# Nablax/Path-Tracer-CUDA-OpenGL

Hardware: AMD Instinct MI355X
Metric: Mray/s + ms/frame, bunny-in-Cornell 1920×1080 @1024spp, 1/2/4/8 MI355X (higher is better)
Workload: dtype f32

## Files before the change

### path-tracer-cuda-opengl_amd/csrc/pt_device.hip

```cpp
#include <hip/hip_runtime.h>

#include <algorithm>
#include <array>
#include <atomic>
#include <chrono>
#include <cfloat>
#include <cmath>
#include <cstdio>
#include <cstdlib>
#include <cstring>
#include <limits>
#include <type_traits>
#include <memory>
#include <string>
#include <vector>

#include "../host/pt_error.hpp"
#include "../host/pt_host.hpp"
#include "../host/pt_inst_dev.hpp"
#include "../host/pt_wide8.hpp"
#include "../host/pt_wide_dev.hpp"
#include "pt.h"
#include "pt_math.hpp"

// ... 55 lines not shown
    uint32_t rays, visits, tris, spheres;
};

__device__ __forceinline__ float3 f3(float a, float b, float c) { return make_float3(a, b, c); }
__device__ __forceinline__ float3 add(float3 a, float3 b) { return f3(a.x + b.x, a.y + b.y, a.z + b.z); }
__device__ __forceinline__ float3 sub(float3 a, float3 b) { return f3(a.x - b.x, a.y - b.y, a.z - b.z); }
__device__ __forceinline__ float3 mul(float3 a, float3 b) { return f3(a.x * b.x, a.y * b.y, a.z * b.z); }
__device__ __forceinline__ float3 scale(float t, float3 v) { return f3(t * v.x, t * v.y, t * v.z); }
__device__ __forceinline__ float3 neg(float3 v) { return f3(-v.x, -v.y, -v.z); }
__device__ __forceinline__ float dot3(float3 a, float3 b) { return a.x * b.x + a.y * b.y + a.z * b.z; }
__device__ __forceinline__ float3 cross3(float3 u, float3 v) {
    return f3(u.y * v.z - u.z * v.y, u.z * v.x - u.x * v.z, u.x * v.y - u.y * v.x);
}
__device__ __forceinline__ float len2(float3 v) { return v.x * v.x + v.y * v.y + v.z * v.z; }
__device__ __forceinline__ float3 divs(float3 v, float t) { return scale(rcpRN(t), v); }
__device__ __forceinline__ float3 normalize3(float3 v) {
    float l = sqrtf(len2(v));
    if (l == 0.0f) return f3(0.0f, 0.0f, 0.0f);
    return divs(v, l);
}
__device__ __forceinline__ float3 xyz(float4 v) { return f3(v.x, v.y, v.z); }

struct Xorwow {
    uint32_t d, v0, v1, v2, v3, v4;
    __device__ __forceinline__ uint32_t next() {
        uint32_t t = v0 ^ (v0 >> 2);
        v0 = v1; v1 = v2; v2 = v3; v3 = v4;
        v4 = __builtin_amdgcn_bitop3_b32(v4, v4 << 4, t ^ (t << 1), 0x96);
        d += 362437u;
        return v4 + d;
    }
    __device__ __forceinline__ float uniform() { return uniformOf(next()); }
    __device__ __forceinline__ float centered2() { return centered2Of(uniform()); }
};

__device__ __forceinline__ Xorwow sampleStream(uint32_t k0, uint32_t k1, uint32_t sample, uint32_t pixel) {
    uint32_t c0 = sample, c1 = pixel, c2 = 0u, c3 = 0x53414D50u;
#pragma unroll 2
    for (int r = 0; r < 10; r++) {
        const uint64_t p0 = (uint64_t)0xD2511F53u * c0, p1 = (uint64_t)0xCD9E8D57u * c2;
        const uint32_t hi0 = (uint32_t)(p0 >> 32), lo0 = (uint32_t)p0;
        const uint32_t hi1 = (uint32_t)(p1 >> 32), lo1 = (uint32_t)p1;
        const uint32_t n0 = __builtin_amdgcn_bitop3_b32(hi1, c1, k0, 0x96), n2 = __builtin_amdgcn_bitop3_b32(hi0, c3, k1, 0x96);
        c0 = n0; c1 = lo1; c2 = n2; c3 = lo0;
        k0 += 0x9E3779B9u;
        k1 += 0xBB67AE85u;
    }
    return Xorwow{c3, c0, c1, c2, c3 ^ 0x6C078965u, c0 ^ c1 ^ 0x2545F491u};
}

struct SlabHit { bool hit; float lo; };

__host__ __device__ constexpr int nodeBoxIdx(int child, int axis, int isMax) { return 6 * child + 2 * axis + isMax; }

typedef float v2f __attribute__((ext_vector_type(2)));

__device__ __forceinline__ SlabHit slabPair(v2f X, v2f Y, v2f Z, float3 o, float3 inv, float tmin, float tmax) {
    const v2f tx = (X - o.x) * inv.x, ty = (Y - o.y) * inv.y, tz = (Z - o.z) * inv.z;
    float nx = inv.x < 0.0f ? tx.y : tx.x, fx = inv.x < 0.0f ? tx.x : tx.y;
    float ny = inv.y < 0.0f ? ty.y : ty.x, fy = inv.y < 0.0f ? ty.x : ty.y;
    float nz = inv.z < 0.0f ? tz.y : tz.x, fz = inv.z < 0.0f ? tz.x : tz.y;
    float lo = fmaxf(fmaxf(fmaxf(tmin, nx), ny), nz);
    float hi = fminf(fminf(fminf(tmax, fx), fy), fz);
    return SlabHit{!(hi < lo), lo};
}
struct SlabHit2 { SlabHit l, r; };
// ... 438 lines not shown
    const float4 s0 = r[0], s1 = r[1], s2 = r[2];
    const uint32_t tf = __float_as_uint(s2.y);
    const bool ident = __float_as_uint(ex.y) == 1u, linIdent = __float_as_uint(ex.y) != 0u;
    HitRec h;
    h.p = add(o, scale(t, d));
    float3 outward;
    if (tf >> 16) {
        const float3 po = ident ? h.p : xformPoint(r0, r1, r2, h.p);
        outward = divs(sub(po, xyz(s0)), s0.w);
    } else {
        outward = xyz(s0);
    }
    if (!linIdent) {
        const float3 n = outward;
        outward = normalize3(f3((r0.x * n.x + r1.x * n.y) + r2.x * n.z, (r0.y * n.x + r1.y * n.y) + r2.y * n.z,
                                (r0.z * n.x + r1.z * n.y) + r2.z * n.z));
    }
    h.front = dot3(d, outward) < 0.0f;
    h.n = h.front ? outward : neg(outward);
    h.mat = (int)__float_as_uint(s2.z);
    obj = (int)(__float_as_uint(ex.x) + __float_as_uint(s2.w));
    h.obj = obj;
    h.m0 = s1;
    h.ir = s2.x;
    h.type = (int)(tf & 0xffffu);
    return h;
}

template <class G>
__device__ __forceinline__ float3 onUnitSphere(G& g) {
    float3 res;
    float norm;
    do {
        const float a = g.centered2();
        const float b = g.centered2();
        const float cz = g.centered2();
        res = f3(a, b, cz);
        norm = len2(res);
    } while (norm >= 1.0f);
    return divs(res, sqrtf(norm));
}
template <class G>
__device__ __forceinline__ float3 inUnitSphere(G& g) {
    float3 res;
    do {
        const float a = g.centered2();
        const float b = g.centered2();
        const float cz = g.centered2();
        res = f3(a, b, cz);
    } while (len2(res) >= 1.0f);
    return res;
}
__device__ __forceinline__ float3 reflect3(float3 v, float3 n) { return sub(v, scale(2.0f * dot3(v, n), n)); }

template <class G>
__device__ __forceinline__ bool scatter(const DevScene& S, const HitRec& h, float3& d, float3& atten, G& g) {
    (void)S;
    const float4 m0 = h.m0;
    const int type = h.type;
    if (type == PT_LAMBERTIAN) {
        float3 dir = add(h.n, onUnitSphere(g));
        if (fabsf(dir.x) < 1e-7f && fabsf(dir.y) < 1e-7f && fabsf(dir.z) < 1e-7f) dir = h.n;
        d = dir;
        atten = xyz(m0);
        return true;
    }
    if (type == PT_METAL) {
        float3 refl = reflect3(normalize3(d), h.n);
        float3 fz = inUnitSphere(g);
        d = add(refl, scale(m0.w, fz));
        atten = xyz(m0);
        return dot3(d, h.n) > 0.0f;
    }
    if (type == PT_DIELECTRIC) {
        atten = f3(1.0f, 1.0f, 1.0f);
        const float ir = h.ir;
        float ratio = h.front ? rcpRN(ir) : ir;
        float3 ud = normalize3(d);
        float cos_t = fminf(dot3(neg(ud), h.n), 1.0f);
        float sin_t = sqrtf(1.0f - cos_t * cos_t);
        bool cannot = ratio * sin_t > 1.0f;
        bool refl = cannot;
// ... 308 lines not shown
#endif
#ifndef PT_LDS_STACK
#define PT_LDS_STACK 32
#endif
template <int STACK, bool SAMPLE, bool WIDE>
constexpr int kLdsStack = (!WIDE && STACK > PT_LDS_STACK) ? PT_LDS_STACK : STACK;
#ifndef PT_WIDE_SPEC
#define PT_WIDE_SPEC 1
#endif
#ifndef PT_WIDE_MIX
#define PT_WIDE_MIX 1
#endif
#ifndef PT_WIDE_WAVES_PER_EU
#define PT_WIDE_WAVES_PER_EU 5
#endif
#ifndef PT_COMPAT_WIDE_WAVES_PER_EU
#define PT_COMPAT_WIDE_WAVES_PER_EU 4
#endif
template <int STACK, bool SAMPLE, bool WIDE>
constexpr int kWavesPerEU = WIDE ? (SAMPLE || STACK > 8 ? PT_WIDE_WAVES_PER_EU : PT_COMPAT_WIDE_WAVES_PER_EU)
                                 : kLdsStack<STACK, SAMPLE, WIDE> <= 24
                                ? (SAMPLE ? PT_WAVES_PER_EU : 5)
                                : (kLdsStack<STACK, SAMPLE, WIDE> <= 32
                                       ? 5
                                       : (kLdsStack<STACK, SAMPLE, WIDE> <= 48 ? 4 : (STACK <= 64 ? 3 : 2)));

typedef const __attribute__((address_space(4))) RenderParams* KArgs;
__device__ __forceinline__ KArgs kargs() {
    KArgs k = (KArgs)__builtin_amdgcn_kernarg_segment_ptr();
    asm volatile("" : "+s"(k));
    return k;
}

typedef const __attribute__((address_space(4))) float KFloat;
typedef const __attribute__((address_space(4))) uint32_t* KU32;
__device__ __forceinline__ float3 ld3(const __attribute__((address_space(4))) float3& v) {
    KFloat* f = (KFloat*)&v;
    return f3(f[0], f[1], f[2]);
}
__device__ __forceinline__ DevScene ldScene(KArgs k) {
    DevScene S;
    S.nodes = k->S.nodes; S.prims = k->S.prims; S.shade = k->S.shade; S.mats = k->S.mats;
    S.wnodes = k->S.wnodes; S.wprims = k->S.wprims; S.wshade = k->S.wshade; S.wbox = k->S.wbox; S.rankOf = k->S.rankOf;
    S.iparent = k->S.iparent; S.err = k->S.err; S.nprims = k->S.nprims;
    S.hasSpheres = k->S.hasSpheres;
    S.cx = k->S.cx; S.cy = k->S.cy; S.cz = k->S.cz; S.ext = k->S.ext;
    S.mixLim = k->S.mixLim;
    S.winst = k->S.winst; S.gBits = k->S.gBits;
    return S;
}

template <bool LIT>
__device__ __forceinline__ float3 skyK(float3 d, float3 att) {
    if constexpr (LIT) return sky(d, att, ld3(kargs()->skyH), ld3(kargs()->skyZ));
    else return sky(d, att);
}

template <int STACK, bool SAMPLE, bool WIDE, bool INST = false, bool LIT = false>
__global__ __launch_bounds__(kWave) __attribute__((amdgpu_waves_per_eu(kWavesPerEU<STACK, SAMPLE, WIDE>))) void renderKernelWF(RenderParams P) {
    constexpr int LS = kLdsStack<STACK, SAMPLE, WIDE>;
    __shared__ uint32_t stk[LS * kWave];
    constexpr int SPECN = WIDE && !INST ? PT_WIDE_SPEC : 0;
    constexpr bool SPEC = SPECN > 0;
    __shared__ uint32_t pend[SPEC ? 2 * SPECN * kWave : 1];
    __shared__ float wray[INST ? 6 * kWave : 1];
    __shared__ uint4 taskState[SAMPLE ? kWave : 1];
// ... 38 lines not shown
    float fcol = (float)col;
    float frow = valid ? (float)globalRow(lrow, P.stripe_h, P.nparts, P.part) : 0.0f;
    const DevScene& S = P.S;
    const __amdgpu_buffer_rsrc_t nodeRsrc = rawRsrc(WIDE ? (const void*)S.wnodes : (const void*)S.nodes);
    uint32_t* my = stk + lane;
    uint32_t sRays = 0, sVisits = 0, sTris = 0, sSph = 0, sPaths = 0;
#ifdef PT_DIAG
    uint32_t itN = 0, itL = 0, itS = 0, sPops = 0, sRedo = 0;
    uint32_t sRedoMiss = 0;
    unsigned long long sSpecN = 0, sIdleN = 0;
    unsigned long long sHalf = 0, sParkT = 0;
    unsigned long long cycN = 0, cycL = 0, cycS = 0, cycH = 0;
    unsigned long long cycSh = 0, cycTk = 0, cycNp = 0, cycBr = 0;
#define PT_DIAG_ADD(v, x) (v) += (x)
#else
#define PT_DIAG_ADD(v, x) ((void)0)
#endif

    Xorwow g{};
    if constexpr (!SAMPLE) {
        if (valid) g = Xorwow{P.sd[idx], P.s0[idx], P.s1[idx], P.s2[idx], P.s3[idx], P.s4[idx]};
    }
    float3 sum = f3(0.0f, 0.0f, 0.0f), o = f3(0.0f, 0.0f, 0.0f), d = f3(0.0f, 0.0f, 1.0f);
    float3 inv = d, att = f3(1.0f, 1.0f, 1.0f);
    float closest = 0.0f;
    int best = -1, depthLeft = 0, sample = 0, node = -1, sp = 0, qn = 0;
    constexpr int LQ = (SAMPLE && !WIDE && STACK <= 32) ? PT_LEAF_QUEUE_SAMPLE : kLeafQ;
    uint32_t qref[LQ];
    float lq[LQ];
#pragma unroll
    for (int i = 0; i < LQ; i++) { qref[i] = 0u; lq[i] = 0.0f; }
    uint32_t ng = 0u, tgBase = 0u, tg = 0u, oct = 0u;
    float bestLo = 0.0f;
    bool active = false;
    uint32_t depthPaths = 0;
    uint32_t pxRays = 0;
    bool needTask = SAMPLE;
    uint32_t poolBase = 0u, poolLeft = 0u;


#define PT_BEGIN_RAY()                                                                              \
    do {                                                                                          \
        depthLeft--;                                                                              \
        if constexpr (SAMPLE) {    \
            if (kargs()->measureCost)                                                             \
                __hip_atomic_fetch_add(&taskState[lane].w, 1u, __ATOMIC_RELAXED, __HIP_MEMORY_SCOPE_WORKGROUP); \
        }                                                                                         \
        closest = __builtin_inff();                                                               \
        best = -1;                                                                                \
        sp = 0;                                                                                   \
        qn = 0;                                                                                   \
        if constexpr (CRITK) pxRays++;                                                            \
        if constexpr (WIDE) {                 \
            inv = f3(rcpRN(d.x), rcpRN(d.y), rcpRN(d.z));                                         \
            const uint32_t oc_ = (inv.x < 0.0f ? 1u : 0u) | (inv.y < 0.0f ? 2u : 0u) | (inv.z < 0.0f ? 4u : 0u); \
            oct = oc_;                                                                            \
            tg = 0u;                                                                              \
                    \
            bestLo = INST || kargs()->S.hasSpheres ? -__builtin_inff() : __builtin_inff();         \
            ng = S.nprims > 0 ? (1u << oc_) : 0u;                                                 \
                 \
            if (!INST && ((kargs()->camFar && depthLeft + 1 == kargs()->max_depth) ||              \
                          (PT_WIDE_MIX && mixUnsafe(inv, kargs()->S.mixLim)))) {                   \
                ng = 0u;             \
                oct |= 8u;      \
            }                                                                                     \
            if (INST && kargs()->camFar && depthLeft + 1 == kargs()->max_depth) {                  \
                     \
                const auto& K_ = *kargs();                                                        \
                (void)instEntry(K_.S.cx, K_.S.cy, K_.S.cz, K_.S.ext, o, d, inv);                   \
// ... 26 lines not shown
                sTris += (uint32_t)__popcll(__ballot(!isS_));                                     \
                sSph += (uint32_t)__popcll(__ballot(isS_));                                       \
                if (sph_) wideTest<true>(q_, o, d, inv, 0.001f, closest, best, bestLo, lb_, redo_, 0u); \
                else if (INST) wideTest<false>(q_, o, d, inv, 0.001f, closest, best, bestLo, lb_, redo_, 0u); \
                else wideTestTri(q_, o, d, 0.001f, closest, best, bestLo);    \
            }                                                                                     \
            if ((ng & 0xffu) == 0u) {                                                             \
                if (sp == 0) break;                                                               \
                sp--;                                                                             \
                ng = my[sp * kWave];                                                              \
            }                                                                                     \
            const uint32_t bit_ = (uint32_t)__builtin_ctz(ng & 0xffu);                            \
            const uint32_t child_ = (ng >> 8) + (bit_ ^ (oct & 7u));                              \
            ng &= ~(1u << bit_);                                                                  \
            if (ng & 0xffu) { my[sp * kWave] = ng; sp++; }    \
            sVisits += (uint32_t)__popcll(__ballot(true));                                        \
            const uint32_t off_ = mul80(child_);                                                  \
            const uint4 n0_ = __builtin_bit_cast(uint4, __builtin_amdgcn_raw_buffer_load_b128(nodeRsrc, off_, 0, 0)); \
            const uint4 n1_ = __builtin_bit_cast(uint4, __builtin_amdgcn_raw_buffer_load_b128(nodeRsrc, off_ + 16u, 0, 0)); \
            const uint4 n2_ = __builtin_bit_cast(uint4, __builtin_amdgcn_raw_buffer_load_b128(nodeRsrc, off_ + 32u, 0, 0)); \
            const uint4 n3_ = __builtin_bit_cast(uint4, __builtin_amdgcn_raw_buffer_load_b128(nodeRsrc, off_ + 48u, 0, 0)); \
            const uint4 n4_ = __builtin_bit_cast(uint4, __builtin_amdgcn_raw_buffer_load_b128(nodeRsrc, off_ + 64u, 0, 0)); \
            const uint32_t h_ = wideHits<PT_WIDE_MIX != 0>(n0_, n1_, n2_, n3_, n4_, o, inv, oct & 7u, 0.001f, closest); \
            ng = (n1_.x << 8) | (h_ >> 24);                                                      \
            tgBase = n1_.y;                                                                       \
            tg = h_ & 0xffffffu;                                                                  \
        }                                                                                         \
        if (redo_) oct |= 8u;              \
    } while (0)
#define PT_TAKE_TASKS(got)                                                                          \
    do {                                                                                          \
        const auto& Q_ = *kargs();                                                                \
        for (;;) {                                                                                \
            const uint64_t m_ = __ballot(needTask);                                               \
            if (m_ == 0) break;                                                                   \
            if (poolLeft == 0u) {  \
                const int leader_ = __ffsll((unsigned long long)m_) - 1;                          \
                          \
                const uint32_t grab_ = (uint32_t)kTaskPool;                                       \
                uint32_t b_ = 0;                                                                  \
                if (lane == leader_) b_ = atomicAdd(Q_.taskCounter, grab_);                       \
                poolBase = __builtin_amdgcn_readfirstlane((uint32_t)__shfl((int)b_, leader_));    \
                poolLeft = grab_;                                                                 \
            }                                                                                     \
              \
            const uint32_t base_ = poolBase;                                                      \
            const uint32_t take_ = min((uint32_t)__popcll(m_), poolLeft);                         \
            poolBase += take_;                                                                    \
            poolLeft -= take_;                                                                    \
            const uint32_t g0_ = base_ >> 6, off_ = base_ & 63u;                                  \
            const uint32_t slotA_ = Q_.nblocksShift >= 0 ? g0_ >> Q_.nblocksShift : g0_ / (uint32_t)Q_.ngroups; \
            const uint32_t blkA_ = g0_ - slotA_ * (uint32_t)Q_.ngroups;                           \
            const bool wrap_ = blkA_ + 1u == (uint32_t)Q_.ngroups;                                  \
            const uint32_t slotB_ = wrap_ ? slotA_ + 1u : slotA_, blkB_ = wrap_ ? 0u : blkA_ + 1u; \
            const uint32_t nslots_ = (uint32_t)Q_.ntiles;                                          \
             \
                                                    \
            const uint32_t xyA_ = slotA_ < nslots_ ? ((KU32)Q_.tileXY)[__builtin_amdgcn_readfirstlane(slotA_)] : 0u; \
            const uint32_t xyB_ = slotB_ < nslots_ ? ((KU32)Q_.tileXY)[__builtin_amdgcn_readfirstlane(slotB_)] : 0u; \
            const uint32_t txA_ = xyA_ & 0xffffu, tyA_ = xyA_ >> 16;                              \
            const uint32_t txB_ = xyB_ & 0xffffu, tyB_ = xyB_ >> 16;                              \
            const uint32_t k_ = (uint32_t)__popcll(m_ & ((1ull << lane) - 1ull));                 \
            if (needTask && k_ < take_) {                                                         \
                if (base_ + k_ >= Q_.ntasks) {                                                     \
                    needTask = false;                                                             \
                } else {                                                                          \
                    const uint32_t o_ = off_ + k_, px_ = o_ & 63u;                                \
                    const bool hi_ = o_ >= 64u;                                                   \
                    const int c_ = (int)((hi_ ? txB_ : txA_) * 8u + (px_ & 7u));                  \
                    const int r_ = (int)((hi_ ? tyB_ : tyA_) * 8u + (px_ >> 3));                  \
                    if (c_ < Q_.width && r_ < Q_.nrows) {                                           \
                        needTask = false;                                                         \
                        got = true;                                                               \
                        const uint32_t s0_ = (hi_ ? blkB_ : blkA_) * (uint32_t)Q_.span;           \
                        taskState[lane] = make_uint4((uint32_t)c_ | ((uint32_t)r_ << 16), s0_,     \
                                                     min(s0_ + (uint32_t)Q_.span, (uint32_t)Q_.spp), 0u); \
                        sum = f3(0.0f, 0.0f, 0.0f);                                               \
                    }                                                                             \
                }                                                                                 \
            }                                                                                     \
        }                                                                                         \
    } while (0)
#define PT_FINISH_TASK(ts)                                                                          \
    do {                                                                                          \
        unsigned long long* acc_ = kargs()->pixAcc + 4 * (size_t)(((ts).x >> 16) * (uint32_t)kargs()->width + ((ts).x & 0xffffu)); \
        addBlock(acc_, sum, (ts).w + 1u, kargs()->measureCost != 0);                              \
        needTask = true;                                                                          \
    } while (0)
#define PT_NEW_PATH()                                                                               \
    do {                                                                                          \
        const auto& Q_ = *kargs();                                                                \
        if constexpr (SAMPLE) {                   \
            const uint4 ts_ = taskState[lane];                                                    \
            fcol = (float)(ts_.x & 0xffffu);                                                      \
            const uint32_t grow_ = (uint32_t)globalRowFast((int)(ts_.x >> 16), Q_.stripe_h, Q_.stripeShift, \
                                                           Q_.nparts, Q_.part);                  \
            frow = (float)grow_;                                                                  \
            g = sampleStream(Q_.seed0, Q_.seed1, Q_.sampleBase + ts_.y,                           \
                             grow_ * (uint32_t)Q_.width + (ts_.x & 0xffffu));                      \
        }                                                                                         \
        const float u_ = (fcol + g.uniform()) * Q_.invW;                                           \
        const float v_ = (frow + g.uniform()) * Q_.invH;                                           \
        o = ld3(Q_.cam.pos);                                                                            \
        d = sub(add(add(ld3(Q_.cam.ll), scale(u_, ld3(Q_.cam.hor))), scale(v_, ld3(Q_.cam.ver))), ld3(Q_.cam.pos));       \
        if (Q_.cam.lens != 0.0f) lensOffset(ld3(Q_.cam.right), ld3(Q_.cam.up), Q_.cam.lens, g, o, d); \
        att = f3(1.0f, 1.0f, 1.0f);                                                               \
        depthLeft = Q_.max_depth;                                                                  \
    } while (0)

#define PT_SKY() skyK<LIT>(d, att)

    bool started = false;
    if constexpr (SAMPLE) {
        if (P.max_depth <= 0) {
            for (;;) {
                bool got = false;
                PT_TAKE_TASKS(got);
                if (__ballot(got) == 0) break;
                if (got) {
                    uint4 ts = taskState[lane];
                    depthPaths += ts.z - ts.y;
                    while (ts.y < ts.z) {
                        taskState[lane].y = ts.y;
                        PT_NEW_PATH();
                        sum = add(sum, PT_SKY());
                        ts.y++;
                        if (ts.y < ts.z) (void)kargs();
                    }
                    PT_FINISH_TASK(ts);
                }
            }
            needTask = false;
            waveReduceAdd(P.counters + 4, depthPaths);
        }
    } else if (valid) {
        if (P.max_depth <= 0) {
            for (; sample < nSamples; sample++) {
                PT_NEW_PATH();
                sum = add(sum, PT_SKY());
            }
        } else if (nSamples > 0) {
            PT_NEW_PATH();
            PT_BEGIN_RAY();
            active = true;
            started = true;
        }
    }
    sRays += (uint32_t)__popcll(__ballot(started));
    sPaths += (uint32_t)__popcll(__ballot(started)) +
              (!SAMPLE && P.max_depth <= 0 ? (uint32_t)__popcll(__ballot(valid)) * (uint32_t)nSamples : 0u);

    for (;;) {
#ifdef PT_DIAG
        const unsigned long long tH0 = __builtin_amdgcn_s_memtime();
#endif
        const bool wantNode = WIDE ? (INST ? ((tg == 0u && ((ng & 0xffu) != 0u || sp > 0)) ||
                                              (SPEC && tg != 0u && (ng & 0xffu) != 0u))
                                           : ((SPEC ? (tg == 0u || ((oct >> 4) & 3u) < (uint32_t)SPECN) : tg == 0u) &&
                                              ((ng & 0xffu) != 0u || sp > 0)))
                                   : (node >= 0 && qn <= LQ - 2);
        const bool wantLeaf = WIDE ? tg != 0u : qn > 0;
        const bool wantShade = (active && (WIDE ? (tg == 0u && (ng & 0xffu) == 0u && sp == 0) : (node == -1 && qn == 0))) ||
                               needTask;
        const uint64_t mN = __ballot(wantNode), mL = __ballot(wantLeaf), mS = __ballot(wantShade);
        if ((mN | mL | mS) == 0) break;
        const int nN = __popcll(mN), nL = __popcll(mL), nS = __popcll(mS);
        int kind;
        if (nN == 0) kind = nL > 0 ? 1 : 2;
        else if (nL >= P.leafBatch) kind = 1;
        else if (nS >= P.shadeBatch) kind = 2;
        else if (!SAMPLE && nN < P.nodeMin && (nL | nS)) kind = nL >= nS ? 1 : 2;
        else kind = 0;
#ifdef PT_DIAG
        const unsigned long long tK0 = __builtin_amdgcn_s_memtime();
        cycH += tK0 - tH0;
#endif

        if (kind == 0) {
            sVisits += (uint32_t)nN;
            PT_DIAG_ADD(itN, 1u);
            if constexpr (WIDE) {
                PT_DIAG_ADD(sSpecN, (unsigned long long)__popcll(__ballot(tg != 0u && ((ng & 0xffu) != 0u || sp > 0))));
                PT_DIAG_ADD(sIdleN, (unsigned long long)(64 - nN));
            }
            if constexpr (INST) {
                if (wantNode) {
                    while ((ng & 0xffu) == 0u && sp > 0) {
                        sp--;
                        ng = my[sp * kWave];
                        if (ng == kInstMarker) {
                            o = f3(wray[0 * kWave + lane], wray[1 * kWave + lane], wray[2 * kWave + lane]);
                            if (oct & 8u) {
                                d = f3(wray[3 * kWave + lane], wray[4 * kWave + lane], wray[5 * kWave + lane]);
                                inv = f3(rcpRN(d.x), rcpRN(d.y), rcpRN(d.z));
                                oct = (inv.x < 0.0f ? 1u : 0u) | (inv.y < 0.0f ? 2u : 0u) | (inv.z < 0.0f ? 4u : 0u);
                            } else {
                                oct &= 7u;
                            }
                            ng = 0u;
                        }
                    }
                    if (ng & 0xffu) {
                        const uint32_t bit = (uint32_t)__builtin_ctz(ng & 0xffu);
                        const uint32_t child = (ng >> 8) + (bit ^ (oct & 7u));
                        ng &= ~(1u << bit);
                        if (ng & 0xffu) { my[sp * kWave] = ng; sp++; }
                        uint32_t off = mul80(child);
                        uint4 n0 = __builtin_bit_cast(uint4, __builtin_amdgcn_raw_buffer_load_b128(nodeRsrc, off, 0, 0));
                        uint4 n1 = __builtin_bit_cast(uint4, __builtin_amdgcn_raw_buffer_load_b128(nodeRsrc, off + 16u, 0, 0));
                        uint4 n2 = __builtin_bit_cast(uint4, __builtin_amdgcn_raw_buffer_load_b128(nodeRsrc, off + 32u, 0, 0));
                        uint4 n3 = __builtin_bit_cast(uint4, __builtin_amdgcn_raw_buffer_load_b128(nodeRsrc, off + 48u, 0, 0));
                        uint4 n4 = __builtin_bit_cast(uint4, __builtin_amdgcn_raw_buffer_load_b128(nodeRsrc, off + 64u, 0, 0));
                        if (n0.w == kInstFlag) {
// ... 1 lines not shown
                            uint32_t full = 0u;
                            if (n0.x == 0u) {
                                const float4 r0 = __builtin_bit_cast(float4, n2), r1 = __builtin_bit_cast(float4, n3),
                                             r2 = __builtin_bit_cast(float4, n4);
                                if (n0.y != 0u) {
                                    o = f3(o.x + r0.w, o.y + r1.w, o.z + r2.w);
                                } else {
                                    wray[3 * kWave + lane] = d.x; wray[4 * kWave + lane] = d.y; wray[5 * kWave + lane] = d.z;
                                    o = xformPoint(r0, r1, r2, o);
                                    d = xformDir(r0, r1, r2, d);
                                    inv = f3(rcpRN(d.x), rcpRN(d.y), rcpRN(d.z));
                                    full = 8u;
                                }
                            }
                            const uint32_t oc = (inv.x < 0.0f ? 1u : 0u) | (inv.y < 0.0f ? 2u : 0u) | (inv.z < 0.0f ? 4u : 0u);
                            my[sp * kWave] = kInstMarker;
                            sp++;
                            oct = oc | full | (n1.y << 8);
                            off = mul80(n1.x);
                            n0 = __builtin_bit_cast(uint4, __builtin_amdgcn_raw_buffer_load_b128(nodeRsrc, off, 0, 0));
                            n1 = __builtin_bit_cast(uint4, __builtin_amdgcn_raw_buffer_load_b128(nodeRsrc, off + 16u, 0, 0));
                            n2 = __builtin_bit_cast(uint4, __builtin_amdgcn_raw_buffer_load_b128(nodeRsrc, off + 32u, 0, 0));
                            n3 = __builtin_bit_cast(uint4, __builtin_amdgcn_raw_buffer_load_b128(nodeRsrc, off + 48u, 0, 0));
                            n4 = __builtin_bit_cast(uint4, __builtin_amdgcn_raw_buffer_load_b128(nodeRsrc, off + 64u, 0, 0));
                        }
                        const uint32_t hits = wideHitsInst(n0, n1, n2, n3, n4, o, inv, oct & 7u, 0.001f, closest);
                        ng = (n1.x << 8) | (hits >> 24);
                        tgBase = n1.y;
                        tg = hits & 0xffffffu;
                    }
                }
            } else if constexpr (WIDE) {
                if (wantNode) {
                    if (SPEC && tg != 0u) {
                        const uint32_t c = SPECN == 1 ? 0u : (oct >> 4) & 3u;
                        pend[(2u * c) * kWave + lane] = tgBase;
                        pend[(2u * c + 1u) * kWave + lane] = tg;
                        oct += 16u;
                    }
                    if constexpr (SPEC) asm volatile("" ::: "memory");
                    if ((ng & 0xffu) == 0u) { sp--; ng = my[sp * kWave]; }
                    const uint32_t bit = (uint32_t)__builtin_ctz(ng & 0xffu);
                    const uint32_t child = (ng >> 8) + (bit ^ (oct & 7u));
                    ng &= ~(1u << bit);
                    if (ng & 0xffu) { my[sp * kWave] = ng; sp++; }
                    const uint32_t off = mul80(child);
                    const uint4 n0 = __builtin_bit_cast(uint4, __builtin_amdgcn_raw_buffer_load_b128(nodeRsrc, off, 0, 0));
                    const uint4 n1 = __builtin_bit_cast(uint4, __builtin_amdgcn_raw_buffer_load_b128(nodeRsrc, off + 16u, 0, 0));
                    const uint4 n2 = __builtin_bit_cast(uint4, __builtin_amdgcn_raw_buffer_load_b128(nodeRsrc, off + 32u, 0, 0));
                    const uint4 n3 = __builtin_bit_cast(uint4, __builtin_amdgcn_raw_buffer_load_b128(nodeRsrc, off + 48u, 0, 0));
                    const uint4 n4 = __builtin_bit_cast(uint4, __builtin_amdgcn_raw_buffer_load_b128(nodeRsrc, off + 64u, 0, 0));
                    const uint32_t hits = wideHits<PT_WIDE_MIX != 0>(n0, n1, n2, n3, n4, o, inv, oct & 7u, 0.001f, closest);
                    ng = (n1.x << 8) | (hits >> 24);
                    tgBase = n1.y;
                    tg = hits & 0xffffffu;
#ifdef PT_DIAG
                    oct &= ~64u;
#endif
                    if (SPEC && tg == 0u && (oct & 48u)) {
                        oct -= 16u;
                        const uint32_t c = SPECN == 1 ? 0u : (oct >> 4) & 3u;
                        tgBase = pend[(2u * c) * kWave + lane];
                        tg = pend[(2u * c + 1u) * kWave + lane];
#ifdef PT_DIAG
                        oct |= 64u;
#endif
                    }
// ... 27 lines not shown
                    for (int i = 0; i < LQ; i++) {
                        qref[i] = qn == i ? rref : qref[i];
                        lq[i] = qn == i ? hr.lo : lq[i];
                    }
                    qn++;
                }
                }
                const bool il = hl.hit && !(lref & kLeafBit), ir = hr.hit && !(rref & kLeafBit);
                if (ir) {
                    if (il) {
                        if (LS == STACK || sp < LS) my[sp * kWave] = lref;
                        else P.stackSpill[((size_t)blockIdx.x * kWave + lane) * (STACK - LS) + (sp - LS)] = lref;
                        sp++;
                    }
                    node = (int)rref;
                } else if (il) {
                    node = (int)lref;
                } else if (sp > 0) {
                    sp--;
                    node = (LS == STACK || sp < LS)
                               ? (int)my[sp * kWave]
                               : (int)P.stackSpill[((size_t)blockIdx.x * kWave + lane) * (STACK - LS) + (sp - LS)];
                } else {
                    node = -1;
                }
            }
        }
        if (kind == 1) {
            bool tested = false, sph = false;
            PT_DIAG_ADD(itL, 1u);
            if constexpr (WIDE) {
                PT_DIAG_ADD(sPops, (uint32_t)nL);
                uint32_t k0 = 0u, k1 = 0u;
                const bool h0 = tg != 0u;
                if (h0) { k0 = tgBase + (uint32_t)__builtin_ctz(tg); tg &= tg - 1u; }
                const bool h1 = tg != 0u;
                if (h1) { k1 = tgBase + (uint32_t)__builtin_ctz(tg); tg &= tg - 1u; }
                const float4* w0 = reinterpret_cast<const float4*>(reinterpret_cast<const char*>(S.wprims) + mul48(k0));
                const float4* w1 = reinterpret_cast<const float4*>(reinterpret_cast<const char*>(S.wprims) + mul48(k1));
                const Prim q0{w0[0], w0[1], w0[2]}, q1{w1[0], w1[1], w1[2]};
                bool redo = false;
#ifdef PT_DIAG
                {
                    sHalf += (unsigned long long)__popcll(__ballot(h0 && !h1));
                    const bool pk = !INST && (oct & 64u) != 0u;
                    sParkT += (unsigned long long)(__popcll(__ballot(pk && h0)) + __popcll(__ballot(pk && h1)));
                }
#endif
                const bool lb = !INST && S.nprims > 1;
                const uint32_t kh = INST ? (oct >> 8) << kargs()->S.gBits : 0u;
                if (kargs()->S.hasSpheres) {
                    if (h0) wideTest<true>(q0, o, d, inv, 0.001f, closest, best, bestLo, lb, redo, kh);
                    if (h1) wideTest<true>(q1, o, d, inv, 0.001f, closest, best, bestLo, lb, redo, kh);
                    const bool s0 = __float_as_uint(q0.p2.w) != 0u, s1 = __float_as_uint(q1.p2.w) != 0u;
                    sTris += (uint32_t)__popcll(__ballot(h0 && !s0)) + (uint32_t)__popcll(__ballot(h1 && !s1));
                    sSph += (uint32_t)__popcll(__ballot(h0 && s0)) + (uint32_t)__popcll(__ballot(h1 && s1));
                } else {
                    if constexpr (INST) {
                        if (h0) wideTest<false>(q0, o, d, inv, 0.001f, closest, best, bestLo, lb, redo, kh);
                        if (h1) wideTest<false>(q1, o, d, inv, 0.001f, closest, best, bestLo, lb, redo, kh);
                    } else {
                        if (h0) wideTestTri(q0, o, d, 0.001f, closest, best, bestLo);
                        if (h1) wideTestTri(q1, o, d, 0.001f, closest, best, bestLo);
                    }
                    sTris += (uint32_t)__popcll(__ballot(h0)) + (uint32_t)__popcll(__ballot(h1));
                }
                if (redo) oct |= 8u;
                if (SPEC && tg == 0u && (oct & 48u)) {
                    oct -= 16u;
                    const uint32_t c = SPECN == 1 ? 0u : (oct >> 4) & 3u;
                    tgBase = pend[(2u * c) * kWave + lane];
                    tg = pend[(2u * c + 1u) * kWave + lane];
#ifdef PT_DIAG
                    oct |= 64u;
#endif
                }
            } else {
            PT_DIAG_ADD(sPops, (uint32_t)nL);
            Prim pf0{}, pf1{};
            if (qn > 0) pf0 = loadPrim(S, qref[0] & kPrimMask);
            if (qn > 1) pf1 = loadPrim(S, qref[1] & kPrimMask);
#pragma unroll
            for (int k_ = 0; k_ < LQ; k_++) {
                const bool act = qn > 0;
                if (__ballot(act) == 0) break;
                tested = false;
                sph = false;
            if (act) {
                const uint32_t ref = qref[0];
                const float lo = lq[0];
#pragma unroll
                for (int i = 0; i + 1 < LQ; i++) { qref[i] = qref[i + 1]; lq[i] = lq[i + 1]; }
                qn--;
                const uint32_t k = ref & kPrimMask;
                sph = (ref & kSphereBit) != 0;
                if (!(closest < lo)) {
                    const Prim pr = k_ == 0 ? pf0 : (k_ == 1 ? pf1 : loadPrim(S, k));
                    {
                        tested = true;
                        const float t = primHitT(pr, sph, o, d, 0.001f, closest);
                        if (t >= 0.0f) { closest = t; best = (int)k; }
                    }
                }
            }
            sTris += (uint32_t)__popcll(__ballot(tested && !sph));
            sSph += (uint32_t)__popcll(__ballot(tested && sph));
            }
            }
        }
        if (kind == 2) {
            if constexpr (WIDE && !INST) {
                bool redo = wantShade && !needTask && (oct & 8u);
#ifdef PT_DIAG
                bool missed = false;
#endif
                if (!kargs()->S.hasSpheres && S.nprims > 1) {
                    if (wantShade && !needTask && best >= 0 && !redo) {
                        const float4* bx = kargs()->S.wbox + 2 * (size_t)best;
                        redo = deferredRedo(bx[0], *reinterpret_cast<const float2*>(bx + 1), o, inv, closest, bestLo);
#ifdef PT_DIAG
                        {
                            const float2 bz_ = *reinterpret_cast<const float2*>(bx + 1);
                            const float4 bx_ = bx[0];
                            missed = !slabPair(v2f{bx_.x, bx_.y}, v2f{bx_.z, bx_.w}, v2f{bz_.x, bz_.y}, o, inv, 0.001f,
                                               __builtin_inff()).hit;
                        }
#endif
                    }
                }
                PT_DIAG_ADD(sRedo, (uint32_t)__popcll(__ballot(redo)));
                PT_DIAG_ADD(sRedoMiss, (uint32_t)__popcll(__ballot(missed)));
                if (redo) {
                    const DevScene S2 = ldScene(kargs());
                    closest = __builtin_inff();
                    const int k = traceRefStackless(S2, o, d, 0.001f, closest);
                    best = k >= 0 ? (int)S2.rankOf[k] : -1;
                }
            }
            bool newRay = false, newSample = false;
            PT_DIAG_ADD(itS, 1u);
            if (wantShade && !needTask) {
                bool done = false;
                float3 contrib = f3(0.0f, 0.0f, 0.0f);
                if (best < 0) {
                    contrib = PT_SKY();
                    done = true;
                } else {
                    int objI_;
                    HitRec h = INST ? makeHitInst(ldScene(kargs()), (uint32_t)best & kPrimMask, closest, o, d, objI_)
                                    : (WIDE ? makeHitFrom(kargs()->S.wshade, best & (int)kPrimMask, closest, o, d)
                                            : makeHit(S, best, closest, o, d));
                    if (!scatterInto(h, d, att, g)) {
                        if constexpr (LIT) contrib = emitted(h, att);
                        done = true;
                    } else {
                        o = h.p;
                        if (depthLeft == 0) { contrib = PT_SKY(); done = true; }
                    }
                }
                if (done) {
                    sum = add(sum, contrib);
                    if constexpr (SAMPLE) {
                        uint4 ts = taskState[lane];
                        ts.y++;
                        taskState[lane].y = ts.y;
                        if (ts.y == ts.z) {
                            active = false;
                            PT_FINISH_TASK(ts);
                        } else {
                            (void)kargs();
                            newSample = true;
                        }
                    } else {
                        ++sample;
                        if (sample == nSamples) {
                            active = false;
                        } else {
                            newSample = true;
                        }
                    }
                }
                newRay = true;
                if (!active) newRay = false;
            }
#ifdef PT_DIAG
            const unsigned long long tS1 = __builtin_amdgcn_s_memtime();
#endif
            if constexpr (SAMPLE) {
                bool got = false;
                PT_TAKE_TASKS(got);
                if (got) {
                    active = true;
                    newRay = newSample = true;
                }
            }
#ifdef PT_DIAG
            const unsigned long long tS2 = __builtin_amdgcn_s_memtime();
#endif
            if (newSample) PT_NEW_PATH();
#ifdef PT_DIAG
            const unsigned long long tS3 = __builtin_amdgcn_s_memtime();
#endif
            if (newRay) PT_BEGIN_RAY();
#ifdef PT_DIAG
            const unsigned long long tS4 = __builtin_amdgcn_s_memtime();
            cycSh += tS1 - tK0; cycTk += tS2 - tS1; cycNp += tS3 - tS2; cycBr += tS4 - tS3;
#endif
            sRays += (uint32_t)__popcll(__ballot(newRay));
            sPaths += (uint32_t)__popcll(__ballot(newSample));
        }
#ifdef PT_DIAG
        {
            const unsigned long long dK = __builtin_amdgcn_s_memtime() - tK0;
            if (kind == 0) cycN += dK;
            else if (kind == 1) cycL += dK;
            else cycS += dK;
        }
#endif
    }
    if constexpr (!SAMPLE) {
        if (valid) {
            storePixel(P, idx, sum);
            P.sd[idx] = g.d; P.s0[idx] = g.v0; P.s1[idx] = g.v1; P.s2[idx] = g.v2; P.s3[idx] = g.v3; P.s4[idx] = g.v4;
            if (CRITK && P.pixRays) P.pixRays[idx] = pxRays;
        }
    }
    const unsigned long long tEnd = __builtin_amdgcn_s_memrealtime();
    if (!SAMPLE && !crit && lane == 0) atomicMax(P.tileCost + tile, (unsigned)min(tEnd - tStart, 0xffffffffull));
    if (P.waveTimes && lane == 0) {
        unsigned xcc;
        asm volatile("s_getreg_b32 %0, hwreg(HW_REG_XCC_ID)" : "=s"(xcc));
        P.waveTimes[3 * (size_t)blockIdx.x + 0] = tStart;
        P.waveTimes[3 * (size_t)blockIdx.x + 1] = tEnd;
        P.waveTimes[3 * (size_t)blockIdx.x + 2] = (unsigned long long)tile | ((unsigned long long)(xcc & 0xf) << 32);
    }
    if (lane == 0) {
        atomicAdd(P.counters + 0, (unsigned long long)sRays);
        atomicAdd(P.counters + 1, (unsigned long long)sVisits);
        atomicAdd(P.counters + 2, (unsigned long long)sTris);
        atomicAdd(P.counters + 3, (unsigned long long)sSph);
        atomicAdd(P.counters + 4, (unsigned long long)sPaths);
#ifdef PT_DIAG
// ... 2778 lines not shown
```

Measured before the change: 20560.

## Track per-lane work state as wave-uniform ballot masks and batch RNG draws

Replaces per-lane booleans (active, needTask, wantNode/Leaf/Shade, got, newRay/newSample) with 64-bit wave masks kept in scalar registers, using inverse_ballot to recover lane predicates. The scheduler loop, task fetch, shading bookkeeping and leaf-pop logic are restructured around these masks, which removes repeated ballots and VGPR-held flags. It also adds a fused three-draw xorwow step for sphere sampling that cuts serial dependencies. The mask bookkeeping is subtle, and divergence from the old semantics (for example the tg sign test in the leaf pop) risks correctness.

```diff
diff --git a/path-tracer-cuda-opengl_amd/csrc/pt_device.hip b/path-tracer-cuda-opengl_amd/csrc/pt_device.hip
--- a/path-tracer-cuda-opengl_amd/csrc/pt_device.hip
+++ b/path-tracer-cuda-opengl_amd/csrc/pt_device.hip
@@ -111,6 +111,21 @@
     }
     __device__ __forceinline__ float uniform() { return uniformOf(next()); }
     __device__ __forceinline__ float centered2() { return centered2Of(uniform()); }
+    __device__ __forceinline__ float3 centered2x3() {
+        uint32_t t0 = v0 ^ (v0 >> 2), t1 = v1 ^ (v1 >> 2), t2 = v2 ^ (v2 >> 2);
+        asm volatile("" : "+v"(t0), "+v"(t1), "+v"(t2));
+        uint32_t r0, r1;
+        asm volatile("v_mov_b32 %0, %1" : "=v"(r0) : "v"(v3));
+        asm volatile("v_mov_b32 %0, %1" : "=v"(r1) : "v"(v4));
+        const uint32_t n0 = __builtin_amdgcn_bitop3_b32(v4, v4 << 4, t0 ^ (t0 << 1), 0x96);
+        const uint32_t n1 = __builtin_amdgcn_bitop3_b32(n0, n0 << 4, t1 ^ (t1 << 1), 0x96);
+        const uint32_t n2 = __builtin_amdgcn_bitop3_b32(n1, n1 << 4, t2 ^ (t2 << 1), 0x96);
+        uint32_t x0 = n0 + (d + 362437u), x1 = n1 + (d + 2u * 362437u);
+        asm volatile("" : "+v"(x0), "+v"(x1));
+        d += 3u * 362437u;
+        v0 = r0; v1 = r1; v2 = n0; v3 = n1; v4 = n2;
+        return f3(centered2Of(uniformOf(x0)), centered2Of(uniformOf(x1)), centered2Of(uniformOf(n2 + d)));
+    }
 };
 
 __device__ __forceinline__ Xorwow sampleStream(uint32_t k0, uint32_t k1, uint32_t sample, uint32_t pixel) {
@@ -615,10 +630,7 @@
     float3 res;
     float norm;
     do {
-        const float a = g.centered2();
-        const float b = g.centered2();
-        const float cz = g.centered2();
-        res = f3(a, b, cz);
+        res = g.centered2x3();
         norm = len2(res);
     } while (norm >= 1.0f);
     return divs(res, sqrtf(norm));
@@ -627,10 +639,7 @@
 __device__ __forceinline__ float3 inUnitSphere(G& g) {
     float3 res;
     do {
-        const float a = g.centered2();
-        const float b = g.centered2();
-        const float cz = g.centered2();
-        res = f3(a, b, cz);
+        res = g.centered2x3();
     } while (len2(res) >= 1.0f);
     return res;
 }
@@ -1005,6 +1014,8 @@
     return k;
 }
 
+__device__ __forceinline__ bool laneOf(uint64_t waveMask) { return __builtin_amdgcn_inverse_ballot_w64(waveMask); }
+
 typedef const __attribute__((address_space(4))) float KFloat;
 typedef const __attribute__((address_space(4))) uint32_t* KU32;
 __device__ __forceinline__ float3 ld3(const __attribute__((address_space(4))) float3& v) {
@@ -1109,10 +1120,11 @@
     for (int i = 0; i < LQ; i++) { qref[i] = 0u; lq[i] = 0.0f; }
     uint32_t ng = 0u, tgBase = 0u, tg = 0u, oct = 0u;
     float bestLo = 0.0f;
-    bool active = false;
+    const uint64_t allM = __ballot(true);
+    uint64_t activeM = 0;
     uint32_t depthPaths = 0;
     uint32_t pxRays = 0;
-    bool needTask = SAMPLE;
+    uint64_t needTaskM = SAMPLE ? allM : 0;
     uint32_t poolBase = 0u, poolLeft = 0u;
 
 
@@ -1205,7 +1217,7 @@
     do {                                                                                          \
         const auto& Q_ = *kargs();                                                                \
         for (;;) {                                                                                \
-            const uint64_t m_ = __ballot(needTask);                                               \
+            const uint64_t m_ = needTaskM;                                                        \
             if (m_ == 0) break;                                                                   \
             if (poolLeft == 0u) {  \
                 const int leader_ = __ffsll((unsigned long long)m_) - 1;                          \
@@ -1234,23 +1246,20 @@
             const uint32_t txA_ = xyA_ & 0xffffu, tyA_ = xyA_ >> 16;                              \
             const uint32_t txB_ = xyB_ & 0xffffu, tyB_ = xyB_ >> 16;                              \
             const uint32_t k_ = (uint32_t)__popcll(m_ & ((1ull << lane) - 1ull));                 \
-            if (needTask && k_ < take_) {                                                         \
-                if (base_ + k_ >= Q_.ntasks) {                                                     \
-                    needTask = false;                                                             \
-                } else {                                                                          \
-                    const uint32_t o_ = off_ + k_, px_ = o_ & 63u;                                \
-                    const bool hi_ = o_ >= 64u;                                                   \
-                    const int c_ = (int)((hi_ ? txB_ : txA_) * 8u + (px_ & 7u));                  \
-                    const int r_ = (int)((hi_ ? tyB_ : tyA_) * 8u + (px_ >> 3));                  \
-                    if (c_ < Q_.width && r_ < Q_.nrows) {                                           \
-                        needTask = false;                                                         \
-                        got = true;                                                               \
-                        const uint32_t s0_ = (hi_ ? blkB_ : blkA_) * (uint32_t)Q_.span;           \
-                        taskState[lane] = make_uint4((uint32_t)c_ | ((uint32_t)r_ << 16), s0_,     \
-                                                     min(s0_ + (uint32_t)Q_.span, (uint32_t)Q_.spp), 0u); \
-                        sum = f3(0.0f, 0.0f, 0.0f);                                               \
-                    }                                                                             \
-                }                                                                                 \
+            const uint32_t o_ = off_ + k_, px_ = o_ & 63u;                                        \
+            const bool hi_ = o_ >= 64u;                                                           \
+            const int c_ = (int)((hi_ ? txB_ : txA_) * 8u + (px_ & 7u));                          \
+            const int r_ = (int)((hi_ ? tyB_ : tyA_) * 8u + (px_ >> 3));                          \
+            const uint64_t took_ = m_ & __ballot(k_ < take_);                                     \
+            const uint64_t left_ = took_ & __ballot(base_ + k_ < Q_.ntasks);                      \
+            const uint64_t in_ = left_ & __ballot(c_ < Q_.width) & __ballot(r_ < Q_.nrows);       \
+            needTaskM &= ~((took_ & ~left_) | in_);                                               \
+            got |= in_;                                                                           \
+            if (laneOf(in_)) {                                                                    \
+                const uint32_t s0_ = (hi_ ? blkB_ : blkA_) * (uint32_t)Q_.span;                   \
+                taskState[lane] = make_uint4((uint32_t)c_ | ((uint32_t)r_ << 16), s0_,             \
+                                             min(s0_ + (uint32_t)Q_.span, (uint32_t)Q_.spp), 0u); \
+                sum = f3(0.0f, 0.0f, 0.0f);                                                       \
             }                                                                                     \
         }                                                                                         \
     } while (0)
@@ -1258,7 +1267,6 @@
     do {                                                                                          \
         unsigned long long* acc_ = kargs()->pixAcc + 4 * (size_t)(((ts).x >> 16) * (uint32_t)kargs()->width + ((ts).x & 0xffffu)); \
         addBlock(acc_, sum, (ts).w + 1u, kargs()->measureCost != 0);                              \
-        needTask = true;                                                                          \
     } while (0)
 #define PT_NEW_PATH()                                                                               \
     do {                                                                                          \
@@ -1287,10 +1295,11 @@
     if constexpr (SAMPLE) {
         if (P.max_depth <= 0) {
             for (;;) {
-                bool got = false;
+                uint64_t got = 0;
                 PT_TAKE_TASKS(got);
-                if (__ballot(got) == 0) break;
-                if (got) {
+                if (got == 0) break;
+                needTaskM |= got;
+                if (laneOf(got)) {
                     uint4 ts = taskState[lane];
                     depthPaths += ts.z - ts.y;
                     while (ts.y < ts.z) {
@@ -1303,7 +1312,7 @@
                     PT_FINISH_TASK(ts);
                 }
             }
-            needTask = false;
+            needTaskM = 0;
             waveReduceAdd(P.counters + 4, depthPaths);
         }
     } else if (valid) {
@@ -1315,27 +1324,34 @@
         } else if (nSamples > 0) {
             PT_NEW_PATH();
             PT_BEGIN_RAY();
-            active = true;
             started = true;
         }
     }
-    sRays += (uint32_t)__popcll(__ballot(started));
-    sPaths += (uint32_t)__popcll(__ballot(started)) +
+    activeM = __ballot(started);
+    sRays += (uint32_t)__popcll(activeM);
+    sPaths += (uint32_t)__popcll(activeM) +
               (!SAMPLE && P.max_depth <= 0 ? (uint32_t)__popcll(__ballot(valid)) * (uint32_t)nSamples : 0u);
 
     for (;;) {
 #ifdef PT_DIAG
         const unsigned long long tH0 = __builtin_amdgcn_s_memtime();
 #endif
-        const bool wantNode = WIDE ? (INST ? ((tg == 0u && ((ng & 0xffu) != 0u || sp > 0)) ||
-                                              (SPEC && tg != 0u && (ng & 0xffu) != 0u))
-                                           : ((SPEC ? (tg == 0u || ((oct >> 4) & 3u) < (uint32_t)SPECN) : tg == 0u) &&
-                                              ((ng & 0xffu) != 0u || sp > 0)))
-                                   : (node >= 0 && qn <= LQ - 2);
-        const bool wantLeaf = WIDE ? tg != 0u : qn > 0;
-        const bool wantShade = (active && (WIDE ? (tg == 0u && (ng & 0xffu) == 0u && sp == 0) : (node == -1 && qn == 0))) ||
-                               needTask;
-        const uint64_t mN = __ballot(wantNode), mL = __ballot(wantLeaf), mS = __ballot(wantShade);
+        uint64_t mN, mL, mS;
+        if constexpr (WIDE) {
+            const uint64_t noPrims = __ballot(tg == 0u);
+            const uint64_t nodesLeft = __ballot(((ng & 0xffu) | (uint32_t)sp) != 0u);
+            uint64_t mayVisit = noPrims;
+            if constexpr (SPEC)
+                mayVisit |= __ballot(SPECN == 1 ? (oct & 48u) == 0u : ((oct >> 4) & 3u) < (uint32_t)SPECN);
+            mN = mayVisit & nodesLeft;
+            mL = allM & ~noPrims;
+            mS = (activeM & noPrims & ~nodesLeft) | needTaskM;
+        } else {
+            const uint64_t inTree = __ballot(node >= 0), queued = __ballot(qn > 0);
+            mN = inTree & (LQ == 2 ? allM & ~queued : __ballot(qn <= LQ - 2));
+            mL = queued;
+            mS = (activeM & ~inTree & ~queued) | needTaskM;
+        }
         if ((mN | mL | mS) == 0) break;
         const int nN = __popcll(mN), nL = __popcll(mL), nS = __popcll(mS);
         int kind;
@@ -1352,6 +1368,7 @@
         if (kind == 0) {
             sVisits += (uint32_t)nN;
             PT_DIAG_ADD(itN, 1u);
+            const bool wantNode = laneOf(mN);
             if constexpr (WIDE) {
                 PT_DIAG_ADD(sSpecN, (unsigned long long)__popcll(__ballot(tg != 0u && ((ng & 0xffu) != 0u || sp > 0))));
                 PT_DIAG_ADD(sIdleN, (unsigned long long)(64 - nN));
@@ -1419,7 +1436,7 @@
                 }
             } else if constexpr (WIDE) {
                 if (wantNode) {
-                    if (SPEC && tg != 0u) {
+                    if (SPEC && laneOf(mL)) {
                         const uint32_t c = SPECN == 1 ? 0u : (oct >> 4) & 3u;
                         pend[(2u * c) * kWave + lane] = tgBase;
                         pend[(2u * c + 1u) * kWave + lane] = tg;
@@ -1513,10 +1530,13 @@
             if constexpr (WIDE) {
                 PT_DIAG_ADD(sPops, (uint32_t)nL);
                 uint32_t k0 = 0u, k1 = 0u;
-                const bool h0 = tg != 0u;
-                if (h0) { k0 = tgBase + (uint32_t)__builtin_ctz(tg); tg &= tg - 1u; }
-                const bool h1 = tg != 0u;
-                if (h1) { k1 = tgBase + (uint32_t)__builtin_ctz(tg); tg &= tg - 1u; }
+                const bool h0 = laneOf(mL);
+                if (h0) k0 = tgBase + (uint32_t)__builtin_ctz(tg);
+                tg &= tg - 1u;
+                const uint64_t m1 = __ballot((int)tg > 0);
+                const bool h1 = laneOf(m1);
+                if (h1) k1 = tgBase + (uint32_t)__builtin_ctz(tg);
+                tg &= tg - 1u;
                 const float4* w0 = reinterpret_cast<const float4*>(reinterpret_cast<const char*>(S.wprims) + mul48(k0));
                 const float4* w1 = reinterpret_cast<const float4*>(reinterpret_cast<const char*>(S.wprims) + mul48(k1));
                 const Prim q0{w0[0], w0[1], w0[2]}, q1{w1[0], w1[1], w1[2]};
@@ -1533,9 +1553,10 @@
                 if (kargs()->S.hasSpheres) {
                     if (h0) wideTest<true>(q0, o, d, inv, 0.001f, closest, best, bestLo, lb, redo, kh);
                     if (h1) wideTest<true>(q1, o, d, inv, 0.001f, closest, best, bestLo, lb, redo, kh);
-                    const bool s0 = __float_as_uint(q0.p2.w) != 0u, s1 = __float_as_uint(q1.p2.w) != 0u;
-                    sTris += (uint32_t)__popcll(__ballot(h0 && !s0)) + (uint32_t)__popcll(__ballot(h1 && !s1));
-                    sSph += (uint32_t)__popcll(__ballot(h0 && s0)) + (uint32_t)__popcll(__ballot(h1 && s1));
+                    const uint64_t s0 = mL & __ballot(__float_as_uint(q0.p2.w) != 0u);
+                    const uint64_t s1 = m1 & __ballot(__float_as_uint(q1.p2.w) != 0u);
+                    sTris += (uint32_t)nL + (uint32_t)__popcll(m1) - (uint32_t)__popcll(s0) - (uint32_t)__popcll(s1);
+                    sSph += (uint32_t)__popcll(s0) + (uint32_t)__popcll(s1);
                 } else {
                     if constexpr (INST) {
                         if (h0) wideTest<false>(q0, o, d, inv, 0.001f, closest, best, bestLo, lb, redo, kh);
@@ -1544,7 +1565,7 @@
                         if (h0) wideTestTri(q0, o, d, 0.001f, closest, best, bestLo);
                         if (h1) wideTestTri(q1, o, d, 0.001f, closest, best, bestLo);
                     }
-                    sTris += (uint32_t)__popcll(__ballot(h0)) + (uint32_t)__popcll(__ballot(h1));
+                    sTris += (uint32_t)nL + (uint32_t)__popcll(m1);
                 }
                 if (redo) oct |= 8u;
                 if (SPEC && tg == 0u && (oct & 48u)) {
@@ -1590,13 +1611,15 @@
             }
         }
         if (kind == 2) {
+            const uint64_t shadeM = mS & ~needTaskM;
+            const bool shading = laneOf(shadeM);
             if constexpr (WIDE && !INST) {
-                bool redo = wantShade && !needTask && (oct & 8u);
+                bool redo = shading && (oct & 8u);
 #ifdef PT_DIAG
                 bool missed = false;
 #endif
                 if (!kargs()->S.hasSpheres && S.nprims > 1) {
-                    if (wantShade && !needTask && best >= 0 && !redo) {
+                    if (shading && best >= 0 && !redo) {
                         const float4* bx = kargs()->S.wbox + 2 * (size_t)best;
                         redo = deferredRedo(bx[0], *reinterpret_cast<const float2*>(bx + 1), o, inv, closest, bestLo);
 #ifdef PT_DIAG
@@ -1618,10 +1641,9 @@
                     best = k >= 0 ? (int)S2.rankOf[k] : -1;
                 }
             }
-            bool newRay = false, newSample = false;
             PT_DIAG_ADD(itS, 1u);
-            if (wantShade && !needTask) {
-                bool done = false;
+            bool done = false;
+            if (shading) {
                 float3 contrib = f3(0.0f, 0.0f, 0.0f);
                 if (best < 0) {
                     contrib = PT_SKY();
@@ -1639,56 +1661,49 @@
                         if (depthLeft == 0) { contrib = PT_SKY(); done = true; }
                     }
                 }
-                if (done) {
-                    sum = add(sum, contrib);
-                    if constexpr (SAMPLE) {
-                        uint4 ts = taskState[lane];
-                        ts.y++;
-                        taskState[lane].y = ts.y;
-                        if (ts.y == ts.z) {
-                            active = false;
-                            PT_FINISH_TASK(ts);
-                        } else {
-                            (void)kargs();
-                            newSample = true;
-                        }
-                    } else {
-                        ++sample;
-                        if (sample == nSamples) {
-                            active = false;
-                        } else {
-                            newSample = true;
-                        }
-                    }
-                }
-                newRay = true;
-                if (!active) newRay = false;
+                if (done) sum = add(sum, contrib);
             }
+            uint64_t doneM, finM;
+            if constexpr (SAMPLE) {
+                const uint4 ts = taskState[lane];
+                const uint32_t y1 = ts.y + (done ? 1u : 0u);
+                taskState[lane].y = y1;
+                doneM = shadeM & __ballot(y1 != ts.y);
+                finM = doneM & __ballot(y1 == ts.z);
+                if (laneOf(finM)) PT_FINISH_TASK(ts);
+                needTaskM |= finM;
+            } else {
+                const int s1 = sample + (done ? 1 : 0);
+                doneM = shadeM & __ballot(s1 != sample);
+                finM = doneM & __ballot(s1 == nSamples);
+                sample = s1;
+            }
+            activeM &= ~finM;
+            uint64_t newRayM = shadeM & ~finM, newSampleM = doneM & ~finM;
 #ifdef PT_DIAG
             const unsigned long long tS1 = __builtin_amdgcn_s_memtime();
 #endif
             if constexpr (SAMPLE) {
-                bool got = false;
+                uint64_t got = 0;
                 PT_TAKE_TASKS(got);
-                if (got) {
-                    active = true;
-                    newRay = newSample = true;
-                }
+                activeM |= got;
+                newRayM |= got;
+                newSampleM |= got;
             }
 #ifdef PT_DIAG
             const unsigned long long tS2 = __builtin_amdgcn_s_memtime();
 #endif
-            if (newSample) PT_NEW_PATH();
+            if (laneOf(newSampleM)) PT_NEW_PATH();
 #ifdef PT_DIAG
             const unsigned long long tS3 = __builtin_amdgcn_s_memtime();
 #endif
-            if (newRay) PT_BEGIN_RAY();
+            if (laneOf(newRayM)) PT_BEGIN_RAY();
 #ifdef PT_DIAG
             const unsigned long long tS4 = __builtin_amdgcn_s_memtime();
             cycSh += tS1 - tK0; cycTk += tS2 - tS1; cycNp += tS3 - tS2; cycBr += tS4 - tS3;
 #endif
-            sRays += (uint32_t)__popcll(__ballot(newRay));
-            sPaths += (uint32_t)__popcll(__ballot(newSample));
+            sRays += (uint32_t)__popcll(newRayM);
+            sPaths += (uint32_t)__popcll(newSampleM);
         }
 #ifdef PT_DIAG
         {
```

Result: faster. 21890 (median of 6 runs) (+6.5%).
